# haasn/libplacebo

Measured on AMD Instinct MI355X. Metric: Mpixels/s (and frames/s) for EWA-Lánczos 1080p→4K + HDR tonemap, 1/2/4/8 GPU, higher is better.
Workload: dtype f32; 1 GPU; ewa_1080p_to_4k_hdr_tonemap; src=1920x1080 rgba16, dst=3840x2160 rgba16, pool=10, api=pl_render_image, measured=output Mpixels/s through pl_render_image, one independent stream per GPU, render_errors=0, parallelism=1 independent stream(s), one per GPU

## Files before the change

libplacebo_amd/csrc/hip/plh_switch.h:

```cpp
#ifndef PLH_SWITCH_H_
#define PLH_SWITCH_H_

#ifdef __cplusplus
extern "C" {
#endif

#define PLH_SWITCHES(X) \
    X(ASYNC_MEASURE,   "PL_HIP_ASYNC_MEASURE",   -1, "0 | 1 override pl_hip_params.async_measure (the measuring pass on a second stream); unset: the parameter") \
    X(NO_FUSION,       "PL_HIP_NO_FUSION",       -1, "1: the renderer records the reference's separate passes; 0: fuses wherever it is valid; unset: where it also pays") \
    X(FUSED_FEATURES,  "PL_HIP_FUSED_FEATURES",   1, "0: the contrast-recovery feature map as its own pass instead of a side output of the plane pass") \
    X(NT_STORE,        "PL_HIP_NT_STORE",         1, "0: plain stores to unorm targets instead of streaming (non-temporal) ones") \
    X(POLAR_MFMA,      "PL_HIP_POLAR_MFMA",       1, "0: every polar pass on the bit-exact sequential-fma kernels instead of the matrix-pipe ones") \
    X(POLAR_PER_PIXEL, "PL_HIP_POLAR_PER_PIXEL",  0, "1: polar weights evaluated per pixel (k_polar) instead of from phase-class tables (k_polar_pp)") \
    X(MX_PERSIST,      "PL_HIP_MX_PERSIST",       1, "0: k_polar_mx (a workgroup per tile) instead of k_polar_mxp (persistent workgroups)") \
    X(MAP_CHAIN,       "PL_HIP_MAP_CHAIN",        1, "0: colour-management ops walked by the interpreter instead of the straight-line chain") \
    X(PQ_SEGMENTS,     "PL_HIP_PQ_SEGMENTS",      1, "0: the chain's PQ pair in closed form instead of piecewise cubics in LDS") \
    X(PQ_SEG_COPIES,   "PL_HIP_PQ_SEG_COPIES",    1, "1 | 2 | 4 | 8 | 16 copies of every piece of those cubics in k_polar_mx's LDS") \
    X(CHAIN_SHAPE,     "PL_HIP_CHAIN_SHAPE",      1, "0: k_polar_mx's generic chain instance always, instead of its shape-specialised one for HDR10 -> SDR passes (bit-identical)") \
    X(PASS_NATIVE,     "PL_HIP_PASS_NATIVE",      1, "0: 1:1 passes on k_pass_generic instead of k_pass_native / k_pass_chain / k_pass_merge / k_pass_mix") \
    X(BILIN_ITERS,     "PL_HIP_BILIN_ITERS",      1, "1 | 2 | 4 cells per lane of k_bilinear_fast; 0: k_pass_generic instead of it and of k_nearest_fast") \
    X(BILIN_TABLES,    "PL_HIP_BILIN_TABLES",     0, "1: the 2x bilinear upscale on k_bilinear_tab (per-axis tables) instead of k_bilinear_fast") \
    X(BILIN_STRIP,     "PL_HIP_BILIN_STRIP",      0, "1: the 2x bilinear upscale on k_bilinear_strip (a 16-byte load per cell) instead of k_bilinear_fast") \
    X(ORTHO_FAST,      "PL_HIP_ORTHO_FAST",       1, "0: separable passes on k_ortho instead of k_ortho_fast") \
    X(LOWPASS_FUSED,   "PL_HIP_LOWPASS_FUSED",    1, "0: the feature map's low-pass as two ortho passes instead of the one k_lowpass2 launch") \
    X(DEBAND_FAST,     "PL_HIP_DEBAND_FAST",      1, "0: debanding on k_deband instead of k_deband_fast / k_deband_lds") \
    X(DEBAND_LDS,      "PL_HIP_DEBAND_LDS",       1, "0: k_deband_fast (fetches from memory) instead of k_deband_lds (window staged in LDS)") \
    X(PEAK_FAST,       "PL_HIP_PEAK_FAST",        1, "0: peak detection on k_pass_peak (the op interpreter) instead of k_peak_tiles / k_peak_fast") \
    X(PEAK_TILES,      "PL_HIP_PEAK_TILES",       1, "0: k_peak_fast + k_peak_fold (two launches) instead of k_peak_tiles (folded on chip)") \
    X(PASS_TRACE,      "PL_HIP_PASS_TRACE",       0, "1: one line per pass launch on stderr: sampler, formats, op list (tools/time_ops.py)") \
    X(PP_ROWS,         "PL_HIP_PP_ROWS",          0, "profiling aid: output rows per lane of k_polar_pp; 0: chosen from the geometry") \
    X(PP_DEBUG,        "PL_HIP_PP_DEBUG",         0, "profiling aid, bit mask: 1 no taps, 2 no verification, 4 no stores, 8 no tile loads")

enum plh_switch_id {
#define PLH_SWITCH_ID(id, name, def, doc) PLH_SW_##id,
    PLH_SWITCHES(PLH_SWITCH_ID)
#undef PLH_SWITCH_ID
    PLH_SW_COUNT
};

int plh_switch(enum plh_switch_id id);

#ifdef __cplusplus
}
#endif

#endif
```

libplacebo_amd/csrc/host/dispatch.c:

```c
#include <math.h>
#include <stdio.h>
#include <stdlib.h>
#include <string.h>

#include <libplacebo/dispatch.h>

#include "shaders_priv.h"

#define MAX_SHADERS 32

struct pass_timing {
    uint64_t signature;
    pl_timer timer;
    struct pl_dispatch_info info;
    int ring;
};

struct pl_dispatch_t {
    pl_log log;
    pl_gpu gpu;
    uint8_t current_ident;
    uint8_t current_index;

    pl_shader pool[MAX_SHADERS];
// ... 712 lines not shown
    return ok;
}

int plh_launch_errdiff(plh_stream stream, const struct plh_errdiff_args *args);

bool pl_dispatch_compute(pl_dispatch dp, const struct pl_dispatch_compute_params *params)
{
    pl_shader sh = *params->shader;
    bool ok = false;

    if (sh->failed) {
        pl_msg(dp->log, PL_LOG_ERR, "Trying to dispatch a failed shader.");
        goto done;
    }
    if (sh->input != PL_SHADER_SIG_NONE) {
        pl_msg(dp->log, PL_LOG_ERR, "Trying to dispatch shader with incompatible signature!");
        goto done;
    }
    if (!pl_shader_is_compute(sh)) {
        pl_msg(dp->log, PL_LOG_ERR, "Trying to dispatch a non-compute shader using "
               "`pl_dispatch_compute`!");
        goto done;
    }

    struct pass_timing *timing = get_timing(dp, sh);
    pl_timer timer = params->timer ? params->timer : timing ? timing->timer : NULL;
    int err;

    if (sh->kind == PLH_SHADER_ERROR_DIFFUSION) {
        if (timer)
            plh_timer_begin(dp->gpu, timer, 0);
        plh_gpu_stamp(dp->gpu, 0);
        err = plh_launch_errdiff(plh_gpu_stream(dp->gpu), sh->errdiff);
        if (timer)
            plh_timer_end(dp->gpu, timer, 0);
    } else {
        if (!params->width || !params->height) {
            pl_msg(dp->log, PL_LOG_ERR, "Trying to dispatch a targetless compute shader "
                   "that uses vertex attributes, this requires specifying the size of the "
                   "effective rendering area!");
            goto done;
        }
        struct plh_pass *pass = &sh->pass;
        memset(&pass->dst, 0, sizeof(pass->dst));
        pass->width = params->width;
        pass->height = params->height;
        pass->out_scale[0] = 1.0 / params->width;
        pass->out_scale[1] = 1.0 / params->height;
        pass->base_x = pass->base_y = 0;
        pass->dir_x = pass->dir_y = 1;
        pass->transpose = 0;
        pass->frag_x0 = pass->frag_y0 = 0;
        plh_pass_choose_cells(pass);
        if (!realize_white_noise(dp->gpu, plh_gpu_stream(dp->gpu), &dp->noise, pass))
            goto done;
        if (timer)
            plh_timer_begin(dp->gpu, timer, 0);
        plh_gpu_stamp(dp->gpu, 0);
        err = plh_launch_pass(plh_gpu_stream(dp->gpu), pass);
        if (timer)
            plh_timer_end(dp->gpu, timer, 0);
        if (!err && sh->detect_peak)
            plh_peak_pass_launched(dp->gpu, sh->peak_state, 0, 0, false);
    }

    if (err) {
        pl_msg(dp->log, PL_LOG_ERR, "Failed launching compute shader '%s': %s",
               sh_description(sh), plh_strerror(err));
        goto done;
    }
    if (!params->timer)
        drain_timing(dp, timing);
    ok = true;

done:
    pl_dispatch_abort(dp, params->shader);
    return ok;
}
```

libplacebo_amd/csrc/host/render_plan.c:

```c
#include <math.h>
#include <stdarg.h>
#include <stdio.h>
#include <stdlib.h>
#include <string.h>

#include "render_plan.h"
#include "host_common.h"


static inline bool rect_unset(const pl_rect2df *rc)
{
    return (!rc->x0 && !rc->x1) || (!rc->y0 && !rc->y1);
}

static void fit_axis(float *s0, float *s1, float *d0, float *d1, float limit)
{
    const bool flip = (*s0 > *s1) != (*d0 > *d1);
    const float slo = PL_MIN(*s0, *s1), shi = PL_MAX(*s0, *s1);
    const float dlo = PL_MIN(*d0, *d1), dhi = PL_MAX(*d0, *d1);

    const float rlo = roundf(PL_CLAMP(dlo, 0.0, limit));
    const float rhi = roundf(PL_CLAMP(dhi, 0.0, limit));

    const float step = (shi - slo) / (dhi - dlo);
// ... 375 lines not shown
    if (pl_color_space_is_hdr(img_color)) {
        st.sigmoid = false;
        if (fbo->type != PL_FMT_FLOAT)
            st.linear = false;
    }
    st.restore_transfer = !st.linear && !st.sigmoid &&
                          img_color->transfer == PL_COLOR_TRC_LINEAR;
    return st;
}


const char *rp_peak_skip_reason(const struct rp_caps *caps, const struct pl_render_params *params,
                                const struct pl_color_space *image, const struct pl_color_space *img,
                                const struct pl_color_space *target)
{
    if (!params->peak_detect_params)
        return "not requested";
    if (!pl_color_space_is_hdr(image))
        return "image is not HDR";
    if (caps->peak_broken)
        return "disabled after an earlier failure";
    if (caps->fbo[4] && !(caps->fbo[4]->caps & PL_FMT_CAP_STORABLE))
        return "intermediate format is not storable";

    float ceiling = pl_color_transfer_nominal_peak(image->transfer) * PL_COLOR_SDR_WHITE;
    if (image->transfer == PL_COLOR_TRC_HLG)
        ceiling = img->hdr.max_luma;
    if (ceiling <= target->hdr.max_luma + 1e-6)
        return "the target covers the image's range";
    if (img->hdr.avg_pq_y)
        return "dynamic metadata already present";

    const struct pl_color_map_params *cm = params->color_map_params;
    const enum pl_hdr_metadata_type wanted = cm ? cm->metadata : PL_HDR_METADATA_ANY;
    if (wanted != PL_HDR_METADATA_ANY && wanted != PL_HDR_METADATA_CIE_Y)
        return "the tone mapper is told to use other metadata";
    if (cm && cm->tone_mapping_function == &pl_tone_map_st2094_40 && img->hdr.ootf.num_anchors)
        return "HDR10+ OOTF in use";
    if (params->lut && params->lut_type == PL_LUT_CONVERSION)
        return "a conversion LUT does the tone mapping";
    return NULL;
}


bool rp_fuse_into_polar(enum rp_direction dir, bool pending_lite, float antiring, int force)
{
    if (force == 1 || dir == RP_DIR_NONE)
        return false;
    if (antiring > 0)
        return false;
    if (force == 0)
        return true;
    return dir == RP_DIR_DOWN || pending_lite;
}

bool rp_wants_feature_map(const struct rp_caps *caps, const struct pl_render_params *params,
                          const struct pl_color_space *img, const struct pl_color_space *target,
                          int out_w, int out_h, int *map_w, int *map_h)
{
    const struct pl_color_map_params *cm = params->color_map_params ? params->color_map_params
                                                                    : &pl_color_map_default_params;
    if (!cm->contrast_recovery || cm->contrast_smoothness <= 1)
        return false;
    if (!caps->fbo[4] || !caps->fbo[1])
        return false;
    if (!pl_color_space_is_hdr(img) || img->hdr.max_luma <= target->hdr.max_luma + 1e-6)
        return false;
    if (caps->sampling_broken || caps->contrast_broken)
        return false;
    if (params->lut && params->lut_type == PL_LUT_CONVERSION)
        return false;
    *map_w = ceilf(out_w / cm->contrast_smoothness);
    *map_h = ceilf(out_h / cm->contrast_smoothness);
    return true;
}


bool rp_wants_blur(const struct pl_render_params *params, const struct pl_frame *target)
{
    const enum pl_clear_mode border = params->skip_target_clearing ? PL_CLEAR_SKIP : params->border;
    return border == PL_CLEAR_BLUR && pl_frame_is_cropped(target);
}

void rp_plan_blur(float radius, int w, int h, struct rp_blur_plan *out)
{
    memset(out, 0, sizeof(*out));
    out->w[0] = w;
    out->h[0] = h;
    if (radius <= 0.0f || (w == 1 && h == 1))
        return;

    const float a_min = 1.0, a_max = 1.8;
    int passes = ceilf(logf(1.0 + radius * radius / (a_max * a_max)) / logf(4.0f));
    passes = PL_CLAMP(passes, 2, RP_MAX_BLUR_PASSES);
    float offset = radius / sqrtf(powf(4, passes) - 1.0f);
    if (offset < a_min && passes > 2)
        offset = radius / sqrtf(powf(4, --passes) - 1.0f);
    if (offset > a_max && passes < RP_MAX_BLUR_PASSES)
        offset = radius / sqrtf(powf(4, ++passes) - 1.0f);

    for (int i = 0; i < passes + 1; i++) {
        out->w[i] = w;
        out->h[i] = h;
        if (w == 1 && h == 1) {
            passes = i;
            break;
// ... 271 lines not shown
```

libplacebo_amd/csrc/host/render_plan.h:

```cpp
#ifndef PLH_RENDER_PLAN_H_
#define PLH_RENDER_PLAN_H_

#include <libplacebo/renderer.h>

struct rp_caps {
    pl_fmt fbo[5];
    size_t max_shmem;
    bool sampling_broken;
    bool peak_broken;
    bool deband_broken;
    bool contrast_broken;
    bool errdiff_broken;
    bool blur_broken;
};

struct rp_geometry {
    pl_rect2df src;
    pl_rect2df dstf;
    pl_rect2d dst;
    pl_rotation rotation;
};

struct rp_geometry rp_fit_rects(pl_rect2df image_crop, int iw, int ih, pl_rotation image_rot,
                                pl_rect2df target_crop, int tw, int th, pl_rotation target_rot);
// ... 32 lines not shown
    float stretch_x, stretch_y;
};

void rp_layout_image(const struct pl_frame *image, struct rp_image_layout *out);
struct pl_sample_src rp_plane_request(const struct rp_image_layout *lay, int i);
bool rp_plane_request_is_identity(const struct pl_sample_src *req);

enum rp_scaler_kind {
    RP_SCALER_BUILTIN = 0,
    RP_SCALER_NEAREST,
    RP_SCALER_BICUBIC,
    RP_SCALER_HERMITE,
    RP_SCALER_GAUSSIAN,
    RP_SCALER_OVERSAMPLE,
    RP_SCALER_FILTER,
};

enum rp_direction { RP_DIR_NONE = 0, RP_DIR_UP, RP_DIR_DOWN };
enum rp_usage { RP_USE_MAIN, RP_USE_PLANE, RP_USE_LOWPASS };

struct rp_scaler {
    enum rp_scaler_kind kind;
    enum rp_direction dir;
    enum rp_direction axis[2];
    const struct pl_filter_config *filter;
};

struct rp_scaler rp_pick_scaler(const struct rp_caps *caps, const struct pl_render_params *params,
                                enum rp_usage usage, const struct pl_sample_src *req,
                                pl_fmt src_format);

struct rp_scale_stage {
    struct rp_scaler scaler;
    bool skip;
    bool defer;
    bool restore_transfer;
    bool linear;
    bool sigmoid;
    bool peak_before;
    int out_w, out_h;
};

struct rp_scale_stage rp_plan_scale(const struct rp_caps *caps, const struct pl_render_params *params,
                                    const struct pl_sample_src *req, pl_fmt src_format,
                                    const struct pl_color_space *img_color, int comps,
                                    bool fixed_size_input);

const char *rp_peak_skip_reason(const struct rp_caps *caps, const struct pl_render_params *params,
                                const struct pl_color_space *image, const struct pl_color_space *img,
                                const struct pl_color_space *target);

bool rp_fuse_into_polar(enum rp_direction dir, bool pending_lite, float antiring, int force);

bool rp_wants_feature_map(const struct rp_caps *caps, const struct pl_render_params *params,
                          const struct pl_color_space *img, const struct pl_color_space *target,
                          int out_w, int out_h, int *map_w, int *map_h);

enum rp_dither { RP_DITHER_NONE = 0, RP_DITHER_ORDERED, RP_DITHER_ERROR_DIFFUSION };

struct rp_output_plane {
    pl_rect2df exact;
    pl_rect2d covered;
    pl_rect2d store;
    struct pl_sample_src request;
    float ratio_x, ratio_y;
};

struct rp_output_stage {
    enum pl_clear_mode background, border;
    bool premultiply;
    bool blend;
    bool drop_alpha;
    bool unpremultiply;
    bool encode;
    bool delinearize_xyz;
    enum pl_lut_type target_lut;
    struct pl_color_repr repr;
    float scale;
    bool transposed;
    pl_rect2d dst;
    bool clear_border;
    int dither_depth;
    int num_planes;
    struct rp_output_plane planes[PL_MAX_PLANES];
};

void rp_plan_output(const struct pl_render_params *params, const struct pl_frame *target,
                    const struct rp_geometry *geo, int img_comps, enum pl_alpha_mode img_alpha,
                    struct rp_output_stage *out);
enum rp_dither rp_pick_dither(const struct rp_caps *caps, const struct pl_render_params *params,
                              int depth, int plane_h);

bool rp_wants_blur(const struct pl_render_params *params, const struct pl_frame *target);

#define RP_MAX_BLUR_PASSES 10
struct rp_blur_plan {
    int passes;
    bool up;
    float offset;
    int w[RP_MAX_BLUR_PASSES + 1], h[RP_MAX_BLUR_PASSES + 1];
};
void rp_plan_blur(float radius, int w, int h, struct rp_blur_plan *out);

struct rp_summary {
    char text[2048];
};
// ... 7 lines not shown
```

libplacebo_amd/csrc/host/renderer.c:

```c
#include <math.h>
#include <stdlib.h>
#include <string.h>

#include <libplacebo/shaders/deinterlacing.h>

#include "renderer_priv.h"

const struct pl_render_params pl_render_fast_params = { PL_RENDER_DEFAULTS };

const struct pl_render_params pl_render_default_params = {
    PL_RENDER_DEFAULTS
    .upscaler           = &pl_filter_lanczos,
    .downscaler         = &pl_filter_hermite,
    .sigmoid_params     = &pl_sigmoid_default_params,
    .dither_params      = &pl_dither_default_params,
    .peak_detect_params = &pl_peak_detect_default_params,
};

const struct pl_render_params pl_render_high_quality_params = {
    PL_RENDER_DEFAULTS
    .upscaler           = &pl_filter_ewa_lanczossharp,
    .downscaler         = &pl_filter_hermite,
    .sigmoid_params     = &pl_sigmoid_default_params,
    .peak_detect_params = &pl_peak_detect_high_quality_params,
// ... 369 lines not shown
                       enum rp_usage usage, const struct pl_sample_src *req)
{
    pl_renderer rr = job->rr;
    const struct pl_render_params *params = job->params;
    struct rp_scaler sc = { .kind = RP_SCALER_BUILTIN };
    if (slot)
        sc = rp_pick_scaler(&job->caps, params, usage, req, req->tex ? req->tex->params.format : NULL);
    if (sc.dir == RP_DIR_NONE)
        sc.kind = RP_SCALER_BUILTIN;

    switch (sc.kind) {
    case RP_SCALER_NEAREST:
        pl_shader_sample_nearest(sh, req);
        return;
    case RP_SCALER_BICUBIC:
        pl_shader_sample_bicubic(sh, req);
        return;
    case RP_SCALER_HERMITE:
        pl_shader_sample_hermite(sh, req);
        return;
    case RP_SCALER_GAUSSIAN:
        pl_shader_sample_gaussian(sh, req);
        return;
    case RP_SCALER_OVERSAMPLE:
        pl_shader_sample_oversample(sh, req, sc.filter->kernel->params[0]);
        return;
    case RP_SCALER_BUILTIN:
        pl_shader_sample_direct(sh, req);
        return;
    case RP_SCALER_FILTER:
        break;
    }

    const struct pl_sample_filter_params fp = {
        .filter      = *sc.filter,
        .antiring    = params->antiringing_strength,
        .no_widening = params->skip_anti_aliasing && usage != RP_USE_LOWPASS,
        .lut         = sc.dir == RP_DIR_UP ? &slot->up : &slot->down,
    };
    bool ok;
    if (sc.filter->polar)
        ok = pl_shader_sample_polar(sh, req, &fp);
    else if (sc.axis[0] && sc.axis[1])
        ok = run_two_pass(job, sh, req, &fp);
    else
        ok = pl_shader_sample_ortho2(sh, req, &fp);

    if (!ok) {
        raise(rr, PL_RENDER_ERR_SAMPLING, PL_LOG_ERR, "Failed dispatching scaler.. disabling");
        pl_shader_sample_direct(sh, req);
    }
}

static bool try_fused_polar(struct frame_job *job, pl_shader sh, const struct pl_sample_src *req,
                            pl_shader pre, int w, int h)
{
    const struct pl_render_params *params = job->params;
    const int force = plh_switch(PLH_SW_NO_FUSION);
    if (!pre || force == 1)
        return false;
    pl_fmt fmt = job->caps.fbo[job->img.comps];
    if (!fmt || fmt->type != PL_FMT_FLOAT || fmt->component_depth[0] != 16)
        return false;

    const struct pl_tex_t stand_in = { .params = { .w = w, .h = h, .format = fmt } };
    struct pl_sample_src probe = *req;
    probe.tex = &stand_in;
    const struct rp_scaler sc = rp_pick_scaler(&job->caps, params, RP_USE_MAIN, &probe, fmt);
    if (sc.kind != RP_SCALER_FILTER || !sc.filter->polar)
        return false;
    bool pending_lite = true;
    for (int i = 0; i < pre->pass.num_ops; i++) {
        switch (pre->pass.ops[i].kind) {
        case PLH_OP_SCALE: case PLH_OP_AFFINE: case PLH_OP_PREMULTIPLY: case PLH_OP_ALPHA_ONE:
        case PLH_OP_QUANT_F16: case PLH_OP_SWIZZLE: case PLH_OP_CLAMP01: case PLH_OP_PLANE_MAP:
            break;
        default:
            pending_lite = false;
        }
    }
    const float ar = sc.filter->antiring ? sc.filter->antiring : params->antiringing_strength;
    if (!rp_fuse_into_polar(sc.dir, pending_lite, ar, force))
        return false;

    const struct pl_sample_filter_params fp = {
        .filter      = *sc.filter,
        .antiring    = params->antiringing_strength,
        .no_widening = params->skip_anti_aliasing,
        .lut         = sc.dir == RP_DIR_UP ? &job->rr->scale_main.up : &job->rr->scale_main.down,
    };
    return plh_shader_sample_polar_fused(sh, pre, &probe, &fp);
}


static void forward_pass_info(void *priv, const struct pl_dispatch_info *dinfo)
{
    struct frame_job *job = priv;
    if (!job->params->info_callback)
        return;
    job->info.pass = dinfo;
    job->params->info_callback(job->params->info_priv, &job->info);
    job->info.index++;
}

void plh_job_watch_passes(struct frame_job *job)
{
    pl_dispatch_reset_frame(job->rr->dp);
    if (job->params->info_callback)
        pl_dispatch_callback(job->rr->dp, job, forward_pass_info);
    else
        pl_dispatch_callback(job->rr->dp, NULL, NULL);
}

bool plh_params_supported(pl_renderer rr, const struct pl_render_params *p)
{
    const char *what = p->num_hooks ? "hooks" : NULL;
    if (!what)
        return true;
    RR_LOG(rr, PL_LOG_ERR, "pl_render_params.%s requests a stage this backend does not have "
           "(outside the pl_render_image hot path, SURVEY.md 8)", what);
    return false;
}

static void note_ignored_members(pl_renderer rr, const struct pl_frame *f)
{
    if ((f->icc || f->profile.data) && !rr->warned_icc) {
        rr->warned_icc = true;
        RR_LOG(rr, PL_LOG_WARN, "ICC profiles are not interpreted by this build (no lcms2): "
               "rendering from the frame's pl_color_space");
    }
    if (f->film_grain.type != PL_FILM_GRAIN_NONE && !rr->warned_grain) {
        rr->warned_grain = true;
        raise(rr, PL_RENDER_ERR_FILM_GRAIN, PL_LOG_WARN,
              "Film grain synthesis is not part of this backend");
    }
}

void plh_job_end(struct frame_job *job)
{
    pl_renderer rr = job->rr;
    pl_dispatch_abort(rr->dp, &job->img.rec);
    pl_dispatch_callback(rr->dp, NULL, NULL);
// ... 377 lines not shown
        .rect  = {
            lay.off_x, lay.off_y,
            lay.off_x + pl_rect_w(lay.planes[lay.ref].rect),
            lay.off_y + pl_rect_h(lay.planes[lay.ref].rect),
        },
        .fail_msg = ref->fail_msg, .fail_bit = ref->fail_bit, .fail_tex = ref->fail_tex,
    };
    struct work_image *img = &job->img;

    const enum pl_lut_type lut = rp_frame_lut_type(image, false);
    const bool raw_lut = lut == PL_LUT_NATIVE || lut == PL_LUT_CONVERSION;
    if (raw_lut) {
        plh_append_scale(sh, pl_color_repr_normalize(&img->repr), true);
        pl_shader_custom_lut(sh, image->lut, &rr->lut_state[RR_LUT_IMAGE]);
    }
    if (lut == PL_LUT_CONVERSION) {
        img->repr.sys = PL_COLOR_SYSTEM_RGB;
        img->repr.levels = PL_COLOR_LEVELS_FULL;
    } else {
        if (img->repr.sys == PL_COLOR_SYSTEM_XYZ) {
            pl_shader_linearize(sh, &img->color);
            img->color.transfer = PL_COLOR_TRC_LINEAR;
        }
        if (img->repr.sys == PL_COLOR_SYSTEM_DOLBYVISION && sh->pass.s.type >= PLH_SAMPLE_POLAR) {
            img->store_as = pl_find_named_fmt(rr->gpu, "rgba32f");
            if (!plh_work_texture(job, img))
                return false;
            sh = plh_work_shader(job, img);
        }
        pl_shader_decode_color(sh, &img->repr, params->color_adjustment);
    }
    if (lut == PL_LUT_NORMALIZED)
        pl_shader_custom_lut(sh, image->lut, &rr->lut_state[RR_LUT_IMAGE]);

    pl_shader_set_alpha(sh, &img->repr, PL_ALPHA_PREMULTIPLIED);
    return !pl_shader_is_failed(sh);
}


static bool owns_workgroup_shape(const pl_shader sh)
{
    const int t = sh->pass.s.type;
    if (t == PLH_SAMPLE_POLAR || t == PLH_SAMPLE_ORTHO || t == PLH_SAMPLE_DEBAND ||
        t == PLH_SAMPLE_DEINTERLACE)
        return true;
    for (int i = 0; i < sh->pass.num_ops; i++) {
        if (sh->pass.ops[i].kind == PLH_OP_DOVI_RESHAPE || sh->pass.ops[i].kind == PLH_OP_DOVI_LMS ||
            sh->pass.ops[i].kind == PLH_OP_CORNER_ROUND)
            return true;
    }
    return false;
}

static void measure_peak(struct frame_job *job)
{
    pl_renderer rr = job->rr;
    const struct pl_render_params *params = job->params;
    struct work_image *img = &job->img;

    const char *why_not = rp_peak_skip_reason(&job->caps, params, &job->image.color, &img->color,
                                              &job->target.color);
    if (!why_not && !job->caps.fbo[4] && !params->peak_detect_params->allow_delayed) {
        raise(rr, PL_RENDER_ERR_PEAK_DETECT, PL_LOG_WARN, "Disabling peak detection because "
              "`pl_peak_detect_params.allow_delayed` is false, but lack of FBOs forces the "
              "result to be delayed.");
        why_not = "no intermediates";
    }
    if (why_not) {
        pl_reset_detected_peak(rr->tone_map_state);
        return;
    }

    if (img->rec && job->caps.fbo[4] && owns_workgroup_shape(img->rec)) {
        pl_tex tex = plh_work_texture(job, img);
        bool ok = tex != NULL;
        if (ok) {
            int mw, mh;
            pl_tex full = NULL;
            if (plh_switch(PLH_SW_FUSED_FEATURES) && !job->features_full &&
                rp_wants_feature_map(&job->caps, params, &img->color, &job->target.color,
                                     abs(pl_rect_w(job->geo.dst)), abs(pl_rect_h(job->geo.dst)), &mw, &mh))
                full = borrow_fbo(job, img->w, img->h, NULL, 1);
            pl_shader probe = pl_dispatch_begin(rr->dp);
            ok = pl_shader_sample_direct(probe, pl_sample_src( .tex = tex )) &&
                 pl_shader_detect_peak(probe, img->color, &rr->tone_map_state,
                                       params->peak_detect_params);
            if (ok && full) {
                pl_shader_extract_features(probe, img->color);
                ok = pl_dispatch_finish(rr->dp, pl_dispatch_params( .shader = &probe, .target = full ));
                if (ok) {
                    job->features_full = full;
                    job->features_src = tex;
                    job->features_color = img->color;
                }
            } else if (ok) {
                ok = pl_dispatch_compute(rr->dp, pl_dispatch_compute_params(
                    .shader = &probe, .width = tex->params.w, .height = tex->params.h,
                ));
            } else {
                pl_dispatch_abort(rr->dp, &probe);
            }
        }
        if (!ok) {
            raise(rr, PL_RENDER_ERR_PEAK_DETECT, PL_LOG_WARN,
                  "Failed measuring the HDR peak.. disabling");
            pl_reset_detected_peak(rr->tone_map_state);
        }
        job->peak_pending = false;
        return;
    }

    if (!pl_shader_detect_peak(plh_work_shader(job, img), img->color, &rr->tone_map_state,
                               params->peak_detect_params)) {
        raise(rr, PL_RENDER_ERR_PEAK_DETECT, PL_LOG_WARN,
              "Failed creating HDR peak detection shader.. disabling");
        pl_reset_detected_peak(rr->tone_map_state);
        return;
    }
    job->peak_pending = !params->peak_detect_params->allow_delayed;
}


bool plh_stage_scale(struct frame_job *job)
{
    pl_renderer rr = job->rr;
    const struct pl_render_params *params = job->params;
    struct work_image *img = &job->img;
    if (!job->caps.fbo[img->comps])
        return true;

    struct pl_sample_src req = {
        .components = img->comps,
        .new_w      = abs(pl_rect_w(job->geo.dst)),
        .new_h      = abs(pl_rect_h(job->geo.dst)),
        .rect       = img->rect,
    };
    int fw, fh;
    const bool fixed = img->rec && pl_shader_output_size(img->rec, &fw, &fh) &&
                       (fw != req.new_w || fh != req.new_h);
    const struct rp_scale_stage st = rp_plan_scale(&job->caps, params, &req, NULL, &img->color,
                                                   img->comps, fixed);
    const pl_rect2df full = { .x1 = st.out_w, .y1 = st.out_h };

    if (st.peak_before)
        measure_peak(job);

    if (st.defer) {
        img->w = st.out_w;
        img->h = st.out_h;
        img->rect = full;
    } else if (!st.skip) {
        if (st.restore_transfer) {
            img->color.transfer = job->image.color.transfer;
            if (img->color.transfer == PL_COLOR_TRC_LINEAR)
                img->color.transfer = PL_COLOR_TRC_GAMMA22;
            pl_shader_delinearize(plh_work_shader(job, img), &img->color);
        }
        if (st.linear || st.sigmoid) {
            pl_shader_linearize(plh_work_shader(job, img), &img->color);
            img->color.transfer = PL_COLOR_TRC_LINEAR;
        }
        if (st.sigmoid)
            pl_shader_sigmoidize(plh_work_shader(job, img), params->sigmoid_params);

        pl_shader sh = pl_dispatch_begin(rr->dp);
        if (img->rec && try_fused_polar(job, sh, &req, img->rec, img->w, img->h)) {
            pl_dispatch_abort(rr->dp, &img->rec);
        } else {
            req.tex = plh_work_texture(job, img);
            if (!req.tex) {
                pl_dispatch_abort(rr->dp, &sh);
                return false;
            }
            run_scaler(job, sh, &rr->scale_main, RP_USE_MAIN, &req);
        }
        job->peak_pending = false;
        img->tex = NULL;
        img->copy_of = NULL;
        img->rec = sh;
        img->w = st.out_w;
        img->h = st.out_h;
        img->rect = full;
        if (st.sigmoid)
            pl_shader_unsigmoidize(sh, params->sigmoid_params);
    }

    if (!st.peak_before)
        measure_peak(job);
    return true;
}


static bool features_color_same(const struct pl_color_space *a, const struct pl_color_space *b)
{
    if (a->primaries != b->primaries || a->transfer != b->transfer)
        return false;
    if (a->transfer == PL_COLOR_TRC_LINEAR || a->transfer == PL_COLOR_TRC_PQ)
        return true;
    return pl_hdr_metadata_equal(&a->hdr, &b->hdr);
}

static pl_tex make_feature_map(struct frame_job *job)
{
    pl_renderer rr = job->rr;
    struct work_image *img = &job->img;
    int mw, mh;
    if (!rp_wants_feature_map(&job->caps, job->params, &img->color, &job->target.color,
                              abs(pl_rect_w(job->geo.dst)), abs(pl_rect_h(job->geo.dst)),
                              &mw, &mh))
        return NULL;
    if (!plh_work_texture(job, img))
        return NULL;

    const bool have = job->features_full && job->features_src == img->tex &&
                      features_color_same(&job->features_color, &img->color);
    pl_tex full = have ? job->features_full : borrow_fbo(job, img->w, img->h, NULL, 1);
    pl_tex small = borrow_fbo(job, mw, mh, NULL, 1);
    bool ok = full && small;
    if (ok && !have) {
        pl_shader sh = pl_dispatch_begin(rr->dp);
        pl_shader_sample_direct(sh, pl_sample_src( .tex = img->tex ));
        pl_shader_extract_features(sh, img->color);
        ok = pl_dispatch_finish(rr->dp, pl_dispatch_params( .shader = &sh, .target = full ));
    }
    if (ok) {
        const struct pl_sample_src req = {
            .tex = full, .rect = img->rect, .address_mode = PL_TEX_ADDRESS_MIRROR,
            .components = 1, .new_w = mw, .new_h = mh,
        };
        if (!try_fused_lowpass(job, &req, small)) {
            pl_shader sh = pl_dispatch_begin(rr->dp);
            run_scaler(job, sh, &rr->scale_contrast, RP_USE_LOWPASS, &req);
            ok = pl_dispatch_finish(rr->dp, pl_dispatch_params( .shader = &sh, .target = small ));
        }
    }
    if (!ok) {
        raise(rr, PL_RENDER_ERR_CONTRAST_RECOVERY, PL_LOG_ERR,
              "Failed extracting luma for contrast recovery, disabling");
        return NULL;
    }
    return small;
// ... 659 lines not shown
    if (!plh_params_supported(rr, params))
        return false;
    if (!pimage)
        return render_nothing(rr, ptarget, params);

    struct pl_render_params local;
    struct pl_peak_detect_params peak;
    if (params->allow_delayed_peak_detect && params->peak_detect_params &&
        !params->peak_detect_params->allow_delayed)
    {
        local = *params;
        peak = *params->peak_detect_params;
        peak.allow_delayed = true;
        local.peak_detect_params = &peak;
        params = &local;
    }

    struct frame_job job = {
        .rr = rr, .params = params, .image = *pimage, .target = *ptarget,
    };
    if (!plh_job_begin(&job, true))
        return false;
    if (!pl_rect_w(job.geo.dst) || !pl_rect_h(job.geo.dst)) {
        plh_job_end(&job);
        return true;
    }

    plh_job_watch_passes(&job);
    bool ok = plh_stage_read(&job) && plh_stage_scale(&job);
    if (ok) {
        plh_stage_colors(&job);
        ok = (job.img.rec || job.img.tex) && plh_stage_output(&job);
    }
    if (!ok)
        RR_LOG(rr, PL_LOG_ERR, "Failed rendering image!");
    plh_job_end(&job);
    return ok;
}

PL_API void plh_test_op_scale(pl_shader sh, float s);
void plh_test_op_scale(pl_shader sh, float s)
{
    struct plh_op *op = sh_op(sh, PLH_OP_SCALE);
    if (op)
        op->f[0] = op->f[1] = op->f[2] = op->f[3] = s;
}

PL_API int plh_test_fuse_into_polar(int dir, int pending_lite, float antiring, int force);
int plh_test_fuse_into_polar(int dir, int pending_lite, float antiring, int force)
{
    return rp_fuse_into_polar((enum rp_direction) dir, pending_lite != 0, antiring, force);
}

PL_API pl_fmt plh_test_format(const char *name);
PL_API size_t plh_test_plan(const struct pl_frame *image, const struct pl_frame *target,
                            const struct pl_render_params *params, bool fbos,
                            size_t max_shmem, char *out, size_t out_size);
size_t plh_test_plan(const struct pl_frame *image, const struct pl_frame *target,
                     const struct pl_render_params *params, bool fbos, size_t max_shmem,
                     char *out, size_t out_size)
{
    struct rp_caps caps = { .max_shmem = max_shmem };
    if (fbos) {
        caps.fbo[4] = caps.fbo[3] = plh_test_format("rgba16hf");
        caps.fbo[2] = plh_test_format("rg16hf");
        caps.fbo[1] = plh_test_format("r16hf");
    }
    struct rp_summary sum;
    rp_summarise(&caps, image, target, params ? params : &pl_render_default_params, &sum);
    const size_t len = strlen(sum.text);
    if (out && out_size) {
        const size_t n = len < out_size - 1 ? len : out_size - 1;
        memcpy(out, sum.text, n);
        out[n] = '\0';
    }
    return len;
}
```

libplacebo_amd/csrc/host/shader_sampling.c:

```c
#include <float.h>
#include <limits.h>
#include <math.h>
#include <stdio.h>
#include <stdlib.h>
#include <string.h>

#include <libplacebo/shaders/sampling.h>

#include "shaders_priv.h"

const struct pl_deband_params pl_deband_default_params = { PL_DEBAND_DEFAULTS };

enum filter_req { REQ_NEAREST, REQ_LINEAR, REQ_BEST, REQ_FASTEST };

struct src_info {
    float ratio_x, ratio_y;
    float scale;
    uint8_t comp_mask;
    bool linear;
};

static bool setup_src(pl_shader sh, const struct pl_sample_src *src, struct src_info *out,
                      bool resizeable, enum filter_req req)
{
// ... 1427 lines not shown
                    const uint16_t hi = f32_to_f16((float) v);
                    const uint16_t lo = f32_to_f16((float) (v - (double) f16_to_f32(hi)));
                    worst = PL_MAX(worst, fabs(v - (double) f16_to_f32(hi) - (double) f16_to_f32(lo)));
                    if (v != 0.0 || vx != 0.0 || vy != 0.0)
                        first_row = PL_MIN(first_row, j);
                    const size_t f = 4 * (size_t) (2 * j + kb);
                    frag[((f + 0) * 64 + l) * 8 + e] = hi;
                    frag[((f + 1) * 64 + l) * 8 + e] = lo;
                    frag[((f + 2) * 64 + l) * 8 + e] = f32_to_f16((float) (vx * dscale));
                    frag[((f + 3) * 64 + l) * 8 + e] = f32_to_f16((float) (vy * dscale));
                }
            }
        }
    }
#undef WN
    free(sx);
    free(sy);
    if (asym > 1e-7) {
        pl_msg(log, PL_LOG_DEBUG, "matrix-pipe downscale: weights not symmetric about the sample "
               "point (%.2e)", asym);
        free(blob);
        return false;
    }
    float *dfx = (float *) (blob + o_dfx), *dfy = (float *) (blob + o_dfy);
    const float up = ldexpf(1.0f, PLH_MX_DSHIFT);
    for (int i = 0; i < W; i++)
        dfx[i] = (colfc[i] - 0.5f) * up;
    for (int i = 0; i < H; i++)
        dfy[i] = (rowfc[i] - 0.5f) * up;

    pl_buf_destroy(gpu, &obj->mx_blob);
    obj->mx_blob = pl_buf_create(gpu, pl_buf_params(.size = bytes, .storable = true,
                                                    .initial_data = blob));
    free(blob);
    if (!obj->mx_blob)
        return false;
    const char *base = pl_hip_buf_ptr(obj->mx_blob);
    obj->mx_host = (struct plh_polar_mx) {
        .enabled = 2,
        .org_x = colbase[0] - 6, .org_y = rowbase[0] - 6,
        .row_first = { first_row, 0 },
        .bfrag = base,
        .dfx = (const float *) (base + o_dfx), .dfy = (const float *) (base + o_dfy),
    };
    obj->mx_announced = false;
    pl_msg(log, PL_LOG_DEBUG, "matrix-pipe tables for the polar pass: 2 : 1 downscale, one phase (1/2, 1/2), "
           "per-pixel phases within %.2e: first-order terms; row symmetry %.1e, weight split error <= %.2e",
           dev, asym, worst);
    return true;
}



bool plh_shader_sample_polar_fused(pl_shader sh, const pl_shader pre,
                                   const struct pl_sample_src *src,
                                   const struct pl_sample_filter_params *params)
{
    const struct plh_pass *pp = &pre->pass;
    pl_tex tex = pre->src_tex;
    if (!tex || pre->failed || pre->kind != PLH_SHADER_PASS || pre->detect_peak)
        return false;
    if (pp->s.type != PLH_SAMPLE_NEAREST && !(pp->s.type == PLH_SAMPLE_BILINEAR && pp->s.rect_on_grid))
        return false;
    const pl_rect2df *rc = &pre->src_rect;
    if (rc->x0 != 0 || rc->y0 != 0 || rc->x1 != tex->params.w || rc->y1 != tex->params.h)
        return false;
    int ow, oh;
    if (pl_shader_output_size(pre, &ow, &oh) && (ow != tex->params.w || oh != tex->params.h))
        return false;
    if (src->tex->params.w != tex->params.w || src->tex->params.h != tex->params.h)
        return false;
    const bool scaled = pp->s.scale != 1.0f;
    if (pp->num_pre_ops || pp->num_ops + scaled > PLH_MAX_OPS - 6)
        return false;
    for (int i = 0; i < pp->num_ops; i++) {
        if (pp->ops[i].kind == PLH_OP_DITHER || pp->ops[i].kind == PLH_OP_PEAK_DETECT ||
            pp->ops[i].kind == PLH_OP_PLANE_FETCH || pp->ops[i].kind == PLH_OP_DOVI_RESHAPE ||
            pp->ops[i].kind == PLH_OP_DOVI_LMS || pp->ops[i].kind == PLH_OP_CORNER_ROUND)
            return false;
    }

    struct pl_sample_src fsrc = *src;
    fsrc.tex = tex;
    fsrc.address_mode = pp->s.address_mode;
    if (!sample_polar(sh, &fsrc, params, true))
        return false;

    struct plh_pass *p = &sh->pass;
    int n = 0;
    if (scaled) {
        struct plh_op *op = &p->ops[n++];
        memset(op, 0, sizeof(*op));
        op->kind = PLH_OP_SCALE;
        op->f[0] = op->f[1] = op->f[2] = op->f[3] = pp->s.scale;
    }
    memcpy(&p->ops[n], pp->ops, pp->num_ops * sizeof(struct plh_op));
    n += pp->num_ops;
    p->num_pre_ops = p->num_ops = n;
    for (int i = 0; i < pre->num_held; i++)
        sh_hold(sh, pre->held[i]);
    sh_listf(sh, "fused_pre_ops(%d ops of '%s' run per source texel, f16 tile)\n", n,
             sh_description(pre));
    return true;
}


enum ortho_axis { ORTHO_VERT = 0, ORTHO_HORIZ = 1 };
static int ortho_axis_of(const struct src_info *info, float *ratio)
{
    const bool keeps_x = fabs(info->ratio_x - 1.0f) < 1e-6f;
    const bool keeps_y = fabs(info->ratio_y - 1.0f) < 1e-6f;
    if (keeps_x) {
        *ratio = info->ratio_y;
        return ORTHO_VERT;
    }
    if (keeps_y) {
        *ratio = info->ratio_x;
        return ORTHO_HORIZ;
    }
    return -1;
}

static struct pl_filter_config effective_filter(const struct pl_sample_filter_params *params, float ratio)
{
    struct pl_filter_config cfg = params->filter;
    float stretch = 1.0 / ratio;
    if (stretch < 1.0f || params->no_widening)
        stretch = 1.0;
    if (!cfg.antiring)
        cfg.antiring = params->antiring;
    cfg.blur = (cfg.blur ? cfg.blur : 1.0f) * stretch;
    return cfg;
}
// ... 212 lines not shown
```

libplacebo_amd/csrc/host/shaders.c:

```c
#include <stdarg.h>
#include <stdio.h>
#include <stdlib.h>
#include <string.h>

#include "shaders_priv.h"


struct info_obj {
    struct pl_shader_info_t pub;
    int refcount;
    char *text;
};

static pl_shader_info info_create(pl_shader sh)
{
    struct info_obj *obj = calloc(1, sizeof(*obj));
    if (!obj)
        return NULL;
    const int n = PL_MAX(sh->num_steps, 1);
    size_t len = 0;
    for (int i = 0; i < sh->num_steps; i++)
        len += strlen(sh->steps[i]) + 1;
    obj->text = calloc(1, 2 * len + 3 * n + 32);
    obj->pub.steps = calloc(n, sizeof(char *));
// ... 343 lines not shown
        return;
    for (int i = 0; i < sh->num_held; i++) {
        if (sh->held[i] == obj)
            return;
    }
    if (sh->num_held >= (int) PL_ARRAY_SIZE(sh->held)) {
        SH_FAIL(sh, "Too many state objects in one shader (%d)", sh->num_held);
        return;
    }
    obj->refcount++;
    sh->held[sh->num_held++] = obj;
}


bool sh_bind(pl_shader sh, pl_tex tex, enum pl_tex_address_mode address_mode,
             const pl_rect2df *rect)
{
    if (pl_tex_params_dimension(tex->params) != 2) {
        SH_FAIL(sh, "Failed binding texture: not a 2D texture!");
        return false;
    }
    if (!tex->params.sampleable) {
        SH_FAIL(sh, "Failed binding texture: texture not sampleable!");
        return false;
    }

    struct plh_sampler_args *s = &sh->pass.s;
    plh_tex_view(tex, &s->src);
    s->address_mode = address_mode;
    sh->src_tex = tex;

    const float sx = 1.0 / tex->params.w, sy = 1.0 / tex->params.h;
    const pl_rect2df full = { .x1 = tex->params.w, .y1 = tex->params.h };
    rect = PL_DEF(rect, &full);
    sh->src_rect = *rect;
    const float x0 = sx * rect->x0, y0 = sy * rect->y0,
                x1 = sx * rect->x1, y1 = sy * rect->y1;
    s->pos[0][0] = x0; s->pos[0][1] = y0;
    s->pos[1][0] = x1; s->pos[1][1] = y0;
    s->pos[2][0] = x0; s->pos[2][1] = y1;
    s->pos[3][0] = x1; s->pos[3][1] = y1;
    s->pt[0] = sx;
    s->pt[1] = sy;
    return true;
}

float plh_fmtf(double v)
{
    char buf[64];
    snprintf(buf, sizeof(buf), "%f", v);
    return strtof(buf, NULL);
}

bool plh_shader_aux_eligible(const pl_shader sh)
{
    if (!sh || sh->failed || sh->kind != PLH_SHADER_PASS || !sh->detect_peak || !sh->src_tex)
        return false;
    const struct plh_pass *p = &sh->pass;
    if (p->s.type != PLH_SAMPLE_NEAREST && p->s.type != PLH_SAMPLE_BILINEAR)
        return false;
    for (int i = 0; i < p->num_ops; i++) {
        const struct plh_op *op = &p->ops[i];
        if (op->kind != PLH_OP_PEAK_DETECT && (op->ptr || op->ptr2))
            return false;
    }
    return true;
}
```

libplacebo_amd/csrc/host/shaders_priv.h:

```cpp
#ifndef PLH_SHADERS_PRIV_H_
#define PLH_SHADERS_PRIV_H_

#include <libplacebo/shaders.h>
#include <libplacebo/shaders/colorspace.h>
#include <libplacebo/colorspace.h>
#include <libplacebo/dispatch.h>

#include "gpu_priv.h"

enum pl_shader_obj_type {
    PL_SHADER_OBJ_INVALID = 0,
    PL_SHADER_OBJ_COLOR_MAP,
    PL_SHADER_OBJ_SAMPLER,
    PL_SHADER_OBJ_DITHER,
    PL_SHADER_OBJ_LUT,
};

struct pl_shader_obj_t {
    int refcount;
    enum pl_shader_obj_type type;
    pl_gpu gpu;
    void (*uninit)(pl_gpu gpu, void *priv);
    void *priv;
};

enum plh_shader_kind {
    PLH_SHADER_PASS = 0,
    PLH_SHADER_ERROR_DIFFUSION,
    PLH_SHADER_BLUR,
};

struct plh_errdiff_args;

struct pl_shader_t {
    pl_log log;
    struct pl_shader_params params;
    bool failed;
    bool mutable_;
    enum pl_shader_sig input, output;
    int output_w, output_h;
    bool transpose;
    bool is_compute;
    int group_size[2];
    size_t shmem;

    enum plh_shader_kind kind;
    struct plh_pass pass;
    pl_shader_obj held[16];
    int num_held;
    bool detect_peak;
    pl_shader_obj peak_state;

    char steps[12][96];
    int num_steps;
    pl_shader_info info;
    char *listing;
    size_t listing_len, listing_cap;
    struct pl_shader_res res;

    uint64_t ticket;

    struct plh_errdiff_args *errdiff;
    struct plh_blur_args blur;
    void *polar_obj;
    pl_tex src_tex;
    pl_rect2df src_rect;
    bool on_aux;
    uint64_t aux_after;
    const void *scratch;
    pl_gpu scratch_gpu;
};

bool plh_shader_aux_eligible(const pl_shader sh);

struct pl_sample_src;
struct pl_sample_filter_params;

bool plh_shader_sample_polar_fused(pl_shader sh, const pl_shader pre,
                                   const struct pl_sample_src *src,
                                   const struct pl_sample_filter_params *params);

struct plh_colormap_plan {
    struct pl_color_space src, dst;
    bool identity;
    struct pl_tone_map_params tone;
    struct pl_gamut_map_params gamut;
    bool closed_form;
    bool need_tone, need_gamut;
    bool tone_direct;
    bool fold_saturation;
};
void plh_colormap_resolve(struct plh_colormap_plan *plan, const struct pl_color_map_params *params,
                                 const struct pl_color_space *src, const struct pl_color_space *dst,
                                 bool stateful);

void plh_polar_pp_setup(pl_gpu gpu, pl_log log, void *polar_obj, struct plh_pass *pass);

void plh_peak_pass_launched(pl_gpu gpu, pl_shader_obj state, int on, uint64_t seq, bool recorded);
plh_event plh_peak_written_event(pl_shader_obj state);

pl_shader plh_shader_from_glsl(const char *glsl);

struct plh_pass_exec {
    struct plh_pass *pass;
    bool transpose;
    void *polar_obj;
    bool detect_peak;
    pl_shader_obj peak_state;
    int out_w, out_h;
    pl_tex src_tex;
    bool on_aux;
    uint64_t aux_after;
};
int plh_pass_execute(pl_gpu gpu, pl_log log, const struct plh_pass_exec *x, pl_tex target,
                     pl_rect2d rc, pl_timer timer, pl_buf *noise);

struct plh_overlay_draw {
    pl_tex tex;
    int mode;
    bool linear;
    bool premultiplied;
    int coverage_at;
    const struct pl_blend_params *blend;
    const struct plh_overlay_part *parts;
    int num_parts;
};
bool plh_dispatch_overlay(pl_dispatch dp, pl_shader *sh, pl_tex target,
                          const struct plh_overlay_draw *draw);
int plh_dispatch_lowpass2(pl_dispatch dp, pl_shader *vert, pl_shader *horiz, pl_tex target);
// ... 36 lines not shown
```

Measured before the change: 90470 Mpixels/s.

## Measure HDR peak in place on a targetless pass before fused polar upscale

```diff
diff --git a/libplacebo_amd/csrc/hip/plh_switch.h b/libplacebo_amd/csrc/hip/plh_switch.h
--- a/libplacebo_amd/csrc/hip/plh_switch.h
+++ b/libplacebo_amd/csrc/hip/plh_switch.h
@@ -8,7 +8,8 @@
 #define PLH_SWITCHES(X) \
     X(ASYNC_MEASURE,   "PL_HIP_ASYNC_MEASURE",   -1, "0 | 1 override pl_hip_params.async_measure (the measuring pass on a second stream); unset: the parameter") \
     X(NO_FUSION,       "PL_HIP_NO_FUSION",       -1, "1: the renderer records the reference's separate passes; 0: fuses wherever it is valid; unset: where it also pays") \
-    X(FUSED_FEATURES,  "PL_HIP_FUSED_FEATURES",   1, "0: the contrast-recovery feature map as its own pass instead of a side output of the plane pass") \
+    X(MEASURE_IN_PLACE, "PL_HIP_MEASURE_IN_PLACE", 1, "0: the HDR measurement in front of a fused polar upscale rides on a pass that writes an rgba16hf copy of the source, instead of reading the source in place") \
+    X(FUSED_FEATURES, "PL_HIP_FUSED_FEATURES",   1, "0: the contrast-recovery feature map as its own pass instead of a side output of the plane pass") \
     X(NT_STORE,        "PL_HIP_NT_STORE",         1, "0: plain stores to unorm targets instead of streaming (non-temporal) ones") \
     X(POLAR_MFMA,      "PL_HIP_POLAR_MFMA",       1, "0: every polar pass on the bit-exact sequential-fma kernels instead of the matrix-pipe ones") \
     X(POLAR_PER_PIXEL, "PL_HIP_POLAR_PER_PIXEL",  0, "1: polar weights evaluated per pixel (k_polar) instead of from phase-class tables (k_polar_pp)") \
diff --git a/libplacebo_amd/csrc/host/dispatch.c b/libplacebo_amd/csrc/host/dispatch.c
--- a/libplacebo_amd/csrc/host/dispatch.c
+++ b/libplacebo_amd/csrc/host/dispatch.c
@@ -788,16 +788,28 @@
         pass->transpose = 0;
         pass->frag_x0 = pass->frag_y0 = 0;
         plh_pass_choose_cells(pass);
-        if (!realize_white_noise(dp->gpu, plh_gpu_stream(dp->gpu), &dp->noise, pass))
+        pl_gpu gpu = dp->gpu;
+        const int on = sh->on_aux && sh->detect_peak && plh_gpu_async(gpu) &&
+                       !plh_gpu_has_peak_exchange(gpu);
+        if (!realize_white_noise(gpu, plh_gpu_stream_n(gpu, on), &dp->noise, pass))
             goto done;
+        uint64_t seq = 0;
+        if (on) {
+            plh_gpu_order_after(gpu, 1, sh->aux_after);
+            seq = plh_tex_order(gpu, 1, sh->src_tex, NULL);
+        } else {
+            plh_gpu_stamp(gpu, 0);
+        }
         if (timer)
-            plh_timer_begin(dp->gpu, timer, 0);
-        plh_gpu_stamp(dp->gpu, 0);
-        err = plh_launch_pass(plh_gpu_stream(dp->gpu), pass);
+            plh_timer_begin(gpu, timer, on);
+        if (sh->detect_peak)
+            plh_launch_offer_stop(plh_peak_written_event(sh->peak_state));
+        err = plh_launch_pass(plh_gpu_stream_n(gpu, on), pass);
+        const bool taken = sh->detect_peak && plh_launch_stop_taken() && !err;
         if (timer)
-            plh_timer_end(dp->gpu, timer, 0);
+            plh_timer_end(gpu, timer, on);
         if (!err && sh->detect_peak)
-            plh_peak_pass_launched(dp->gpu, sh->peak_state, 0, 0, false);
+            plh_peak_pass_launched(gpu, sh->peak_state, on, seq, taken);
     }
 
     if (err) {
diff --git a/libplacebo_amd/csrc/host/render_plan.c b/libplacebo_amd/csrc/host/render_plan.c
--- a/libplacebo_amd/csrc/host/render_plan.c
+++ b/libplacebo_amd/csrc/host/render_plan.c
@@ -451,6 +451,19 @@
     if (force == 0)
         return true;
     return dir == RP_DIR_DOWN || pending_lite;
+}
+
+bool rp_measure_in_place(const struct rp_measure_site *site, int fusion, int enabled)
+{
+    if (!enabled)
+        return false;
+    if (!site->before_scaler)
+        return false;
+    if (site->stage_adds_ops)
+        return false;
+    if (!site->plain_fetch || !site->fbo_f16 || !site->polar_main)
+        return false;
+    return rp_fuse_into_polar(site->dir, site->pending_lite, site->antiring, fusion);
 }
 
 bool rp_wants_feature_map(const struct rp_caps *caps, const struct pl_render_params *params,
diff --git a/libplacebo_amd/csrc/host/render_plan.h b/libplacebo_amd/csrc/host/render_plan.h
--- a/libplacebo_amd/csrc/host/render_plan.h
+++ b/libplacebo_amd/csrc/host/render_plan.h
@@ -108,6 +108,18 @@
 
 bool rp_fuse_into_polar(enum rp_direction dir, bool pending_lite, float antiring, int force);
 
+struct rp_measure_site {
+    bool before_scaler;
+    bool stage_adds_ops;
+    bool polar_main;
+    enum rp_direction dir;
+    bool plain_fetch;
+    bool pending_lite;
+    bool fbo_f16;
+    float antiring;
+};
+bool rp_measure_in_place(const struct rp_measure_site *site, int fusion, int enabled);
+
 bool rp_wants_feature_map(const struct rp_caps *caps, const struct pl_render_params *params,
                           const struct pl_color_space *img, const struct pl_color_space *target,
                           int out_w, int out_h, int *map_w, int *map_h);
diff --git a/libplacebo_amd/csrc/host/renderer.c b/libplacebo_amd/csrc/host/renderer.c
--- a/libplacebo_amd/csrc/host/renderer.c
+++ b/libplacebo_amd/csrc/host/renderer.c
@@ -445,42 +445,62 @@
     }
 }
 
-static bool try_fused_polar(struct frame_job *job, pl_shader sh, const struct pl_sample_src *req,
-                            pl_shader pre, int w, int h)
+struct polar_boundary {
+    struct rp_scaler sc;
+    struct pl_tex_t stand_in;
+    bool fbo_f16;
+    bool pending_lite;
+    float antiring;
+};
+
+static void probe_polar_boundary(const struct frame_job *job, const struct pl_sample_src *req,
+                                 const pl_shader pre, int w, int h, struct polar_boundary *b)
 {
     const struct pl_render_params *params = job->params;
-    const int force = plh_switch(PLH_SW_NO_FUSION);
-    if (!pre || force == 1)
-        return false;
+    memset(b, 0, sizeof(*b));
     pl_fmt fmt = job->caps.fbo[job->img.comps];
-    if (!fmt || fmt->type != PL_FMT_FLOAT || fmt->component_depth[0] != 16)
-        return false;
-
-    const struct pl_tex_t stand_in = { .params = { .w = w, .h = h, .format = fmt } };
+    b->fbo_f16 = fmt && fmt->type == PL_FMT_FLOAT && fmt->component_depth[0] == 16;
+    if (!b->fbo_f16)
+        return;
+    b->stand_in = (struct pl_tex_t) { .params = { .w = w, .h = h, .format = fmt } };
     struct pl_sample_src probe = *req;
-    probe.tex = &stand_in;
-    const struct rp_scaler sc = rp_pick_scaler(&job->caps, params, RP_USE_MAIN, &probe, fmt);
-    if (sc.kind != RP_SCALER_FILTER || !sc.filter->polar)
-        return false;
-    bool pending_lite = true;
+    probe.tex = &b->stand_in;
+    b->sc = rp_pick_scaler(&job->caps, params, RP_USE_MAIN, &probe, fmt);
+    b->pending_lite = true;
     for (int i = 0; i < pre->pass.num_ops; i++) {
         switch (pre->pass.ops[i].kind) {
         case PLH_OP_SCALE: case PLH_OP_AFFINE: case PLH_OP_PREMULTIPLY: case PLH_OP_ALPHA_ONE:
         case PLH_OP_QUANT_F16: case PLH_OP_SWIZZLE: case PLH_OP_CLAMP01: case PLH_OP_PLANE_MAP:
             break;
         default:
-            pending_lite = false;
-        }
-    }
-    const float ar = sc.filter->antiring ? sc.filter->antiring : params->antiringing_strength;
-    if (!rp_fuse_into_polar(sc.dir, pending_lite, ar, force))
-        return false;
-
+            b->pending_lite = false;
+        }
+    }
+    if (b->sc.kind == RP_SCALER_FILTER)
+        b->antiring = b->sc.filter->antiring ? b->sc.filter->antiring : params->antiringing_strength;
+}
+
+static bool try_fused_polar(struct frame_job *job, pl_shader sh, const struct pl_sample_src *req,
+                            pl_shader pre, int w, int h)
+{
+    const struct pl_render_params *params = job->params;
+    const int force = plh_switch(PLH_SW_NO_FUSION);
+    if (!pre || force == 1)
+        return false;
+    struct polar_boundary b;
+    probe_polar_boundary(job, req, pre, w, h, &b);
+    if (!b.fbo_f16 || b.sc.kind != RP_SCALER_FILTER || !b.sc.filter->polar)
+        return false;
+    if (!rp_fuse_into_polar(b.sc.dir, b.pending_lite, b.antiring, force))
+        return false;
+
+    struct pl_sample_src probe = *req;
+    probe.tex = &b.stand_in;
     const struct pl_sample_filter_params fp = {
-        .filter      = *sc.filter,
+        .filter      = *b.sc.filter,
         .antiring    = params->antiringing_strength,
         .no_widening = params->skip_anti_aliasing,
-        .lut         = sc.dir == RP_DIR_UP ? &job->rr->scale_main.up : &job->rr->scale_main.down,
+        .lut         = b.sc.dir == RP_DIR_UP ? &job->rr->scale_main.up : &job->rr->scale_main.down,
     };
     return plh_shader_sample_polar_fused(sh, pre, &probe, &fp);
 }
@@ -964,7 +984,30 @@
     return false;
 }
 
-static void measure_peak(struct frame_job *job)
+static bool measures_in_place(struct frame_job *job, const struct rp_scale_stage *st,
+                              const struct pl_sample_src *req)
+{
+    const struct work_image *img = &job->img;
+    if (!st || !img->rec || img->rec->kind != PLH_SHADER_PASS)
+        return false;
+    struct polar_boundary b;
+    probe_polar_boundary(job, req, img->rec, img->w, img->h, &b);
+    const struct rp_measure_site site = {
+        .before_scaler  = st->peak_before && !st->skip && !st->defer,
+        .stage_adds_ops = st->restore_transfer || st->linear || st->sigmoid,
+        .polar_main     = b.sc.kind == RP_SCALER_FILTER && b.sc.filter->polar,
+        .dir            = b.sc.dir,
+        .plain_fetch    = plh_polar_fusable(img->rec, img->w, img->h),
+        .pending_lite   = b.pending_lite,
+        .fbo_f16        = b.fbo_f16,
+        .antiring       = b.antiring,
+    };
+    return rp_measure_in_place(&site, plh_switch(PLH_SW_NO_FUSION),
+                               plh_switch(PLH_SW_MEASURE_IN_PLACE));
+}
+
+static void measure_peak(struct frame_job *job, const struct rp_scale_stage *st,
+                         const struct pl_sample_src *req)
 {
     pl_renderer rr = job->rr;
     const struct pl_render_params *params = job->params;
@@ -1022,6 +1065,28 @@
         return;
     }
 
+    if (measures_in_place(job, st, req)) {
+        pl_shader probe = pl_dispatch_begin(rr->dp);
+        bool ok = plh_shader_copy_recording(probe, img->rec) &&
+                  pl_shader_detect_peak(probe, img->color, &rr->tone_map_state,
+                                        params->peak_detect_params);
+        if (ok) {
+            probe->on_aux = plh_gpu_async(rr->gpu) && plh_shader_aux_eligible(probe);
+            ok = pl_dispatch_compute(rr->dp, pl_dispatch_compute_params(
+                .shader = &probe, .width = img->w, .height = img->h,
+            ));
+        } else {
+            pl_dispatch_abort(rr->dp, &probe);
+        }
+        if (!ok) {
+            raise(rr, PL_RENDER_ERR_PEAK_DETECT, PL_LOG_WARN,
+                  "Failed measuring the HDR peak.. disabling");
+            pl_reset_detected_peak(rr->tone_map_state);
+        }
+        job->peak_pending = false;
+        return;
+    }
+
     if (!pl_shader_detect_peak(plh_work_shader(job, img), img->color, &rr->tone_map_state,
                                params->peak_detect_params)) {
         raise(rr, PL_RENDER_ERR_PEAK_DETECT, PL_LOG_WARN,
@@ -1055,7 +1120,7 @@
     const pl_rect2df full = { .x1 = st.out_w, .y1 = st.out_h };
 
     if (st.peak_before)
-        measure_peak(job);
+        measure_peak(job, &st, &req);
 
     if (st.defer) {
         img->w = st.out_w;
@@ -1098,7 +1163,7 @@
     }
 
     if (!st.peak_before)
-        measure_peak(job);
+        measure_peak(job, NULL, NULL);
     return true;
 }
 
@@ -1864,6 +1929,17 @@
     return rp_fuse_into_polar((enum rp_direction) dir, pending_lite != 0, antiring, force);
 }
 
+PL_API int plh_test_measure_in_place(const int *site, float antiring, int fusion, int enabled);
+int plh_test_measure_in_place(const int *site, float antiring, int fusion, int enabled)
+{
+    const struct rp_measure_site s = {
+        .before_scaler = site[0] != 0, .stage_adds_ops = site[1] != 0, .polar_main = site[2] != 0,
+        .dir = (enum rp_direction) site[3], .plain_fetch = site[4] != 0,
+        .pending_lite = site[5] != 0, .fbo_f16 = site[6] != 0, .antiring = antiring,
+    };
+    return rp_measure_in_place(&s, fusion, enabled);
+}
+
 PL_API pl_fmt plh_test_format(const char *name);
 PL_API size_t plh_test_plan(const struct pl_frame *image, const struct pl_frame *target,
                             const struct pl_render_params *params, bool fbos,
diff --git a/libplacebo_amd/csrc/host/shader_sampling.c b/libplacebo_amd/csrc/host/shader_sampling.c
--- a/libplacebo_amd/csrc/host/shader_sampling.c
+++ b/libplacebo_amd/csrc/host/shader_sampling.c
@@ -1503,9 +1503,7 @@
 
 
 
-bool plh_shader_sample_polar_fused(pl_shader sh, const pl_shader pre,
-                                   const struct pl_sample_src *src,
-                                   const struct pl_sample_filter_params *params)
+bool plh_polar_fusable(const pl_shader pre, int w, int h)
 {
     const struct plh_pass *pp = &pre->pass;
     pl_tex tex = pre->src_tex;
@@ -1519,7 +1517,7 @@
     int ow, oh;
     if (pl_shader_output_size(pre, &ow, &oh) && (ow != tex->params.w || oh != tex->params.h))
         return false;
-    if (src->tex->params.w != tex->params.w || src->tex->params.h != tex->params.h)
+    if (w != tex->params.w || h != tex->params.h)
         return false;
     const bool scaled = pp->s.scale != 1.0f;
     if (pp->num_pre_ops || pp->num_ops + scaled > PLH_MAX_OPS - 6)
@@ -1530,6 +1528,18 @@
             pp->ops[i].kind == PLH_OP_DOVI_LMS || pp->ops[i].kind == PLH_OP_CORNER_ROUND)
             return false;
     }
+    return true;
+}
+
+bool plh_shader_sample_polar_fused(pl_shader sh, const pl_shader pre,
+                                   const struct pl_sample_src *src,
+                                   const struct pl_sample_filter_params *params)
+{
+    if (!plh_polar_fusable(pre, src->tex->params.w, src->tex->params.h))
+        return false;
+    const struct plh_pass *pp = &pre->pass;
+    pl_tex tex = pre->src_tex;
+    const bool scaled = pp->s.scale != 1.0f;
 
     struct pl_sample_src fsrc = *src;
     fsrc.tex = tex;
diff --git a/libplacebo_amd/csrc/host/shaders.c b/libplacebo_amd/csrc/host/shaders.c
--- a/libplacebo_amd/csrc/host/shaders.c
+++ b/libplacebo_amd/csrc/host/shaders.c
@@ -419,6 +419,34 @@
     return strtof(buf, NULL);
 }
 
+bool plh_shader_copy_recording(pl_shader sh, const pl_shader from)
+{
+    if (!from || from->failed || !from->mutable_ || from->kind != PLH_SHADER_PASS ||
+        from->detect_peak || from->polar_obj || from->scratch)
+        return false;
+    if (sh->failed || !sh->mutable_ || sh->output != PL_SHADER_SIG_NONE || sh->num_held)
+        return false;
+    sh->input = from->input;
+    sh->output = from->output;
+    sh->output_w = from->output_w;
+    sh->output_h = from->output_h;
+    sh->transpose = from->transpose;
+    sh->is_compute = from->is_compute;
+    sh->group_size[0] = from->group_size[0];
+    sh->group_size[1] = from->group_size[1];
+    sh->shmem = from->shmem;
+    sh->pass = from->pass;
+    sh->src_tex = from->src_tex;
+    sh->src_rect = from->src_rect;
+    memcpy(sh->steps, from->steps, sizeof(sh->steps));
+    sh->num_steps = from->num_steps;
+    for (size_t at = 0; from->listing && at < from->listing_len; at += 500)
+        sh_listf(sh, "%.500s", from->listing + at);
+    for (int i = 0; i < from->num_held; i++)
+        sh_hold(sh, from->held[i]);
+    return !sh->failed;
+}
+
 bool plh_shader_aux_eligible(const pl_shader sh)
 {
     if (!sh || sh->failed || sh->kind != PLH_SHADER_PASS || !sh->detect_peak || !sh->src_tex)
diff --git a/libplacebo_amd/csrc/host/shaders_priv.h b/libplacebo_amd/csrc/host/shaders_priv.h
--- a/libplacebo_amd/csrc/host/shaders_priv.h
+++ b/libplacebo_amd/csrc/host/shaders_priv.h
@@ -73,8 +73,12 @@
 
 bool plh_shader_aux_eligible(const pl_shader sh);
 
+bool plh_shader_copy_recording(pl_shader sh, const pl_shader from);
+
 struct pl_sample_src;
 struct pl_sample_filter_params;
+
+bool plh_polar_fusable(const pl_shader pre, int w, int h);
 
 bool plh_shader_sample_polar_fused(pl_shader sh, const pl_shader pre,
                                    const struct pl_sample_src *src,
```

New measurement: 89840 Mpixels/s. No clear change (-0.7%).
